# WdBlink/pyflyt-drone

Hardware: AMD Instinct MI355X
Metric: env-steps/sec at N parallel envs (FixedwingWaypoints) (higher is better)
Workload: dtype f64

## Files before the change

include/fwsim.h:

```cpp
#ifndef FWSIM_H
#define FWSIM_H

#include <stdint.h>

#ifdef __cplusplus
extern "C" {
#endif

#define FW_ABI_VERSION 7

#define FW_NUM_SURFACES 5
#define FW_NUM_ACTUATORS 6
#define FW_MAX_TARGETS 8
#define FW_MAX_COLLISION_PTS 8
#define FW_MAX_OBSTACLES 20
#define FW_VISION_FEATS 9
#define FW_VISION_HIST 3

enum {
  FW_OK = 0,
  FW_EINVAL = -1,
  FW_EHIP = -2,
  FW_ENOMEM = -3,
  FW_EVERSION = -4,
// ... 411 lines not shown
  void* act_env;
  float *rew_out, *start_out;
  void *obs, *reward;
  uint8_t *terminated, *truncated;
  void* terminal_obs;
  int32_t* info_i32;
  void* workspace; int64_t workspace_bytes;
  void* trace;
  double gamma;
  float clip_obs, eps_obs, clip_reward, eps_reward;
  int32_t update_obs, update_ret, norm_reward, deterministic;
} fw_collect_args;
int64_t fw_collect_step_workspace_bytes(fw_handle h);
int32_t fw_collect_workspace_init(fw_handle h, void* workspace, int64_t workspace_bytes, void* hip_stream);
int32_t fw_collect_step(fw_handle h, const fw_collect_args* a, void* hip_stream);
int32_t fw_collect_finish(fw_handle h, const fw_collect_args* a, void* hip_stream);
int32_t fw_collect_status(fw_handle h, const void* workspace, int64_t workspace_bytes, uint32_t* status_out, void* hip_stream);
typedef struct fw_collect_close_args {
  const float *rewards, *values, *episode_starts;
  float *adv, *ret;
  int32_t T;
  float gae_gamma, gae_lambda;
} fw_collect_close_args;
int32_t fw_collect_close(fw_handle h, const fw_collect_args* a, const fw_collect_close_args* c, void* hip_stream);

int32_t fw_num_envs(fw_handle h);
int32_t fw_lanes_per_env(fw_handle h);
int32_t fw_capture_wave(fw_handle h);
int32_t fw_axis_aligned(fw_handle h);
int32_t fw_aux_wave(fw_handle h);
int32_t fw_step_shape(fw_handle h);
enum {
  FW_PROBE_MATH1 = 0, FW_PROBE_MATH2 = 1, FW_PROBE_ROT = 2, FW_PROBE_EULER = 3, FW_PROBE_QUAT_STEP = 4, FW_PROBE_SURFACE = 5,
  FW_PROBE_GROUP = 6, FW_PROBE_RNG = 7, FW_PROBE_WIND = 8
};
enum { FW_PROBE_EULER_LANE = 0, FW_PROBE_EULER_LANES8 = 1, FW_PROBE_EULER_INVERSE = 2 };
enum { FW_PROBE_SURFACE_SCALAR = 0, FW_PROBE_SURFACE_REGS = 1, FW_PROBE_SURFACE_LDS = 2, FW_PROBE_SURFACE_AX = 3 };
enum { FW_PROBE_RNG_PHILOX = 0, FW_PROBE_RNG_UNIFORM = 1, FW_PROBE_RNG_NORMAL2 = 2 };
int32_t fw_probe(fw_handle h, int32_t op, int32_t variant, const double* in, int32_t in_cols, double* out, int32_t out_cols,
                 int32_t n, void* hip_stream);
typedef struct fw_sac_hyper {
  float lr, gamma, tau, beta1, beta2, eps, target_entropy, ent_coef;
  int32_t auto_ent, target_update_interval;
  uint64_t seed;
} fw_sac_hyper;
int32_t fw_sizeof_sac_hyper(void);
int32_t fw_sac_param_count(int32_t obs_dim, int32_t act_dim, int32_t hidden);
int64_t fw_sac_update_workspace_bytes(int32_t obs_dim, int32_t act_dim, int32_t hidden, int32_t batch);
int32_t fw_sac_act(const float* image, const void* obs, int32_t obs_is_f64, int32_t N, int32_t obs_dim, int32_t act_dim, int32_t hidden, int32_t mode,
                   uint64_t seed, int64_t env_offset, const int64_t* counters, float* act_f32, void* act_env, float* obs_stage, float* logp,
                   float* eps, void* hip_stream);
int32_t fw_replay_store(float* ring, int64_t capacity, int64_t* counters, const float* obs_stage, const float* act_f32, const void* reward,
                        const void* next_obs, const void* terminal_obs, const uint8_t* terminated, const uint8_t* truncated, int32_t env_is_f64,
                        int32_t N, int32_t obs_dim, int32_t act_dim, void* hip_stream);
int32_t fw_replay_sample(const float* ring, int64_t capacity, const int64_t* counters, uint64_t seed, int32_t row_floats, int32_t batch,
                         float* out, int32_t* idx_out, void* hip_stream);
int32_t fw_sac_noise(uint64_t seed, const int64_t* counters, int32_t batch, int32_t act_dim, float* out, void* hip_stream);
int32_t fw_sac_update(float* image, const float* batch_rows, int32_t obs_dim, int32_t act_dim, int32_t hidden, int32_t batch, const fw_sac_hyper* hyper,
                      int64_t* counters, float* out, void* workspace, int64_t workspace_bytes, void* hip_stream);
const char* fw_last_error(fw_handle h);
int32_t fw_destroy(fw_handle h);

#ifdef __cplusplus
}
#endif
#endif
```

pyflyt-drone_amd/csrc/fwsim.hip:

```cpp
#include <hip/hip_runtime.h>

#include <algorithm>
#include <cmath>
#include <cstdio>
#include <cstdlib>
#include <cstring>
#include <map>
#include <mutex>
#include <new>
#include <string>
#include <type_traits>
#include <vector>

#include "fwsim_device.hpp"
#include "fwsim_rollout.hpp"
#include "fwsim_ppo.hpp"
#include "fwsim_collect.hpp"
#include "fwsim_fused.hpp"
#include "fwsim_objlock.hpp"
#include "fwsim_render.hpp"

using namespace fwsim;


// ... 4 lines not shown
  for (int f = 0; f < RF_COUNT; ++f) D.r[tile_index(tile, RF_COUNT, f, env)] = (T)0;
  D.r[tile_index(tile, RF_COUNT, RF_QUAT + 3, env)] = (T)1;
  for (int f = 0; f < IF_COUNT; ++f) D.i[tile_index(tile, IF_COUNT, f, env)] = 0;
  D.i[tile_index(tile, IF_COUNT, IF_FLAGS, env)] = FL_TERM;
  D.i[tile_index(tile, IF_COUNT, IF_EPISODE, env)] = -1;
}

template <typename T>
__global__ void fw_warm_kernel(Params<T>* Pm) {
  if (threadIdx.x != 0 || blockIdx.x != 0) return;
  const Params<T>& P = *Pm;
  Rigid<T> S;
  for (int k = 0; k < 3; ++k) { S.p[k] = P.start_pos[k]; S.v[k] = P.start_vel[k]; S.w[k] = (T)0; }
  for (int k = 0; k < 4; ++k) S.q[k] = P.start_quat[k];
  for (int k = 0; k < FW_NUM_ACTUATORS; ++k) S.act[k] = (T)0;
  T cmd0[FW_NUM_ACTUATORS] = {(T)0, (T)0, (T)0, (T)0, (T)0, (T)0};
  T wind0[3] = {(T)0, (T)0, (T)0};
  int ticks = P.warmup_aviary_steps * P.ticks_per_aviary;
  TickC<T> C; SurfC<T> mine; T wmask;
  load_tick_constants<T, 1>(Pm, C, mine, wmask);
  T R[9];
  normalize_quat<T>(S.q);
  rot_from_unit_quat<T>(S.q, R);
  LaneAct<T> LA; LA.a = (T)0; LA.cmd = (T)0;
  for (int t = 0; t < ticks; ++t) (void)physics_tick<T, false, 1>(P, C, S, R, cmd0, (T)0, wind0, mine, wmask, LA);
  for (int k = 0; k < 3; ++k) { Pm->warm[k] = S.p[k]; Pm->warm[7 + k] = S.v[k]; Pm->warm[10 + k] = S.w[k]; }
  for (int k = 0; k < 4; ++k) Pm->warm[3 + k] = S.q[k];
  for (int k = 0; k < FW_NUM_ACTUATORS; ++k) Pm->warm[13 + k] = S.act[k];
  Pm->warm_ticks = ticks;
  const T a0[4] = {(T)0, (T)0, (T)0, (T)0};
  T Rw[9];
  (void)write_obs_attitude<T, false>(P, S, a0, Rw, [&](int k, T v) { Pm->warm_obs[k] = v; });
  for (int k = 0; k < 9; ++k) Pm->warm_R[k] = Rw[k];
}

__device__ __forceinline__ void pf_issue(double& dst, const double* p) { asm volatile("global_load_dwordx2 %0, %1, off" : "=v"(dst) : "v"(p) : "memory"); }
__device__ __forceinline__ void pf_issue(float& dst, const float* p) { asm volatile("global_load_dword %0, %1, off" : "=v"(dst) : "v"(p) : "memory"); }
template <typename T> __device__ __forceinline__ void pf_wait(T& a, T& b, T& c, T& d) { asm volatile("s_waitcnt vmcnt(0)" : "+v"(a), "+v"(b), "+v"(c), "+v"(d) :: "memory"); }
template <typename T> __device__ __forceinline__ void pf_tie(T& a, T& b, T& c, T& d) { asm volatile("" : "+v"(a), "+v"(b), "+v"(c), "+v"(d)); }
template <typename T> __device__ __forceinline__ T vload(const T* p) { return *p; }

template <typename T, bool COH = false>
__device__ __forceinline__ void load_action(const DevState<T>& D, const T* actions, int env, int src, T a[4]) {
  const T* ap = actions + (size_t)env * 4;
#pragma unroll
  for (int k = 0; k < 4; ++k) {
    T cur = COH ? ld_coherent(ap + k) : ap[k], old = D.r[(size_t)(RF_ACTION + k) * D.npad + env];
    a[k] = (src == 0) ? cur : (src == 1) ? old : (T)0;
  }
}

template <typename T> __device__ __forceinline__ DevState<T> shadow_view(const DevState<T>& D) {
  DevState<T> V = D; V.r = D.rs; V.i = nullptr; return V;
}
__device__ __forceinline__ unsigned long long pack_done(uint32_t ep, uint32_t epoch, int done) {
  return ((unsigned long long)ep << 32) | ((unsigned long long)(epoch & 0xFFFFFFu) << 8) | (unsigned long long)(done & 0xFF);
}

template <typename T, int G, int TKIND>
__device__ __forceinline__ void shadow_worker(const Params<T>* __restrict__ Pp, const ObjC<T>* __restrict__ OCp, DevState<T> D, int blk, int max_chunk = 0) {
  constexpr bool OBJ = TKIND == FW_TASK_OBJLOCK, COMB = TKIND == FW_TASK_WAYPOINT_OBJLOCK, HASOBJ = OBJ || COMB;
  constexpr int EPW = kWave / G;
  const Params<T>& P = *Pp;
  const ObjC<T>& OC = *OCp;
  const int lane = threadIdx.x & (kWave - 1), sub = (G == 1) ? 0 : (lane & (G - 1)), row = lane / G;
  const bool leader = sub == 0;
// ... 181 lines not shown

  T* aux_nz = AUX ? reinterpret_cast<T*>(smem_raw + Dg.mbox_off) : nullptr;
  if constexpr (AUX) {
    if (threadIdx.x >= kWave) {
      const int32_t a_tick = D.i[IF_TICK * n + envc], a_episode = D.i[IF_EPISODE * n + envc], a_flags = D.i[IF_FLAGS * n + envc];
      T a_z0 = (T)0, a_z1 = (T)0;
      if (FW_SH(has_noise) && FW_SH(step_ratio) <= G && !(a_flags & (FL_TERM | FL_TRUNC)))
        rng_normal2<T>(P, (uint32_t)(P.env_offset + envc), (uint32_t)a_episode, (uint32_t)(a_tick / FW_SH(ticks_per_aviary)) + (uint32_t)sub, a_z0, a_z1);
      aux_nz[2 * lane] = a_z0; aux_nz[2 * lane + 1] = a_z1;
      __syncthreads();
      return;
    }
  }

  int32_t step_count = D.i[IF_STEP * n + envc];
  int32_t tick = D.i[IF_TICK * n + envc];
  int32_t episode = D.i[IF_EPISODE * n + envc];
  int32_t flags = D.i[IF_FLAGS * n + envc];
  int32_t num_reached = D.i[IF_NUM_REACHED * n + envc];
  constexpr bool LANE_T = DEFER && G == 8;
  T tmine[3] = {(T)0, (T)0, (T)0};
  T a_keep = (T)0;
  if (LANE_T) {
    if (sub < FW_SH(num_targets)) {
#pragma unroll
      for (int k = 0; k < 3; ++k) tmine[k] = D.r[(size_t)(RF_TARGETS + 3 * sub + k) * n + envc];
    }
    if (!COLLECT) a_keep = actions[(size_t)envc * 4 + (sub & 3)];
  }
  Rigid<T> S;
  load_rigid<T>(D, envc, S);
  T new_dist = D.r[RF_NEW_DIST * n + envc];
  T ep_return = D.r[RF_EP_RETURN * n + envc];
  TickC<T> C; SurfC<T> mine_regs; T wmask;
  load_tick_constants<T, G, DEFER && G == 8 && WPE == 1>(Pp, C, mine_regs, wmask);
  if (AX && sub >= FW_NUM_SURFACES) mine_regs.hra = (T)0;
  SurfC<T>& mine = mine_regs;

  normalize_quat<T>(S.q);
  T R[9];
  rot_from_unit_quat<T>(S.q, R);
  ObjState<T> O;
  const ObjC<T>& OC = *OCp;
  if (HASOBJ) { obj_load<T, OBJ>(D, envc, O); obj_update_near_mask<T, G>(P, OC, D, envc, O, S); }
  int32_t out_strike = 0;
  unsigned long long sh_req = ~0ull, sh_done = 0ull;
  if ((GENERAL || DEFER) && D.shadow_on) { sh_req = D.sreq[envc]; sh_done = D.sdone[envc]; }
  T wb[3] = {(T)0, (T)0, (T)0}, wa[3] = {(T)0, (T)0, (T)0}, wphase = (T)0;
  if (GENERAL) {
#pragma unroll
    for (int k = 0; k < 3; ++k) { wb[k] = D.r[(RF_WIND + k) * n + envc]; wa[k] = D.r[(RF_WIND + 3 + k) * n + envc]; }
    wphase = D.r[(RF_WIND + 6) * n + envc];
  }
  T gust[2] = {(T)0, (T)1};
  if (GENERAL) gust_init<T>(P, wphase, tick, gust);
  T rew = (T)-0.1;
  T cmd[FW_NUM_ACTUATORS];
  double c_ret = 0.0;
  if (COLLECT) {
    if (active && leader) c_ret = ld_sc1(CAp->S.returns + env);
    collect_wait_actions(*CAp, Dg.epoch, env0, min(EPW, Dg.n - env0));
  }
  {
    const T* ap = actions + (size_t)envc * 4;
    T a4[4];
    if (COLLECT) collect_load_actions<T>(*CAp, ap, a4);
    else {
#pragma unroll
      for (int k = 0; k < 4; ++k) a4[k] = ap[k];
    }
    if (COLLECT && LANE_T) a_keep = (sub & 3) == 0 ? a4[0] : (sub & 3) == 1 ? a4[1] : (sub & 3) == 2 ? a4[2] : a4[3];
    const T sp[4] = { a4[0], a4[1], a4[2], a4[3] * (T)0.5 + (T)0.5 };
#pragma unroll
    for (int c = 0; c < FW_NUM_ACTUATORS; ++c)
      cmd[c] = P.mixer[c][0] * sp[0] + P.mixer[c][1] * sp[1] + P.mixer[c][2] * sp[2] + P.mixer[c][3] * sp[3];
  }
  LaneAct<T> LA; LA.a = (T)0; LA.cmd = (T)0;
  T cmd_mine = (T)0;
  if (G == 8) { lane_act_scatter<T>(S, LA); cmd_mine = lane_pick5<T>(cmd[0], cmd[1], cmd[2], cmd[3], cmd[4]); LA.cmd = cmd_mine; }

  T tcur[3] = {(T)0, (T)0, (T)0}, tnext[3] = {(T)0, (T)0, (T)0};
  const int gbase = lane & ~(G - 1);
  if (LANE_T) {
#pragma unroll
    for (int k = 0; k < 3; ++k) tcur[k] = __shfl(tmine[k], gbase | (num_reached & (G - 1)), kWave);
  } else if (!OBJ) {
    const int i0 = min(num_reached, FW_MAX_TARGETS - 1), i1 = min(num_reached + 1, FW_MAX_TARGETS - 1);
#pragma unroll
    for (int k = 0; k < 3; ++k) {
      tcur[k] = D.r[(size_t)(RF_TARGETS + 3 * i0 + k) * n + envc];
      tnext[k] = D.r[(size_t)(RF_TARGETS + 3 * i1 + k) * n + envc];
    }
  }

  const uint32_t genv = (uint32_t)(P.env_offset + envc);
  const bool done_at_entry = (flags & (FL_TERM | FL_TRUNC)) != 0;
  int tgt_obs = (flags >> FL_TGT_SHIFT) & 15;
  flags &= FL_MASK;
  int act_src = done_at_entry ? 1 : 0;

  const uint32_t astep0 = (uint32_t)(tick / FW_SH(ticks_per_aviary));
  const bool pre_noise = (G == 8) && FW_SH(has_noise) && (FW_SH(step_ratio) <= G);
  T nz0 = (T)0, nz1 = (T)0;
  if (!AUX && pre_noise && !done_at_entry) rng_normal2<T>(P, genv, (uint32_t)episode, astep0 + (uint32_t)sub, nz0, nz1);

  int phase = active ? PH_STEP : PH_DONE;
  constexpr bool STASH = (!DEFER && !HASOBJ) || COLLECT;
  double* latch = STASH ? reinterpret_cast<double*>(smem_raw + Dg.stash_off) : nullptr;
  int it = 0, warm_left = 0;
  const Mbox<T> MB = mbox_at<T>(HELP ? Dg.mbox_off : 0);
  uint32_t n_posted = 0, pend_seq = 0;
  int pend = 0;
// ... 1356 lines not shown
  O.near_ = (T)c.camera_near; O.far_ = (T)c.camera_far;
  O.inv_near = (T)(1.0 / c.camera_near); O.inv_far = (T)(1.0 / c.camera_far); O.db_c1 = (T)(c.camera_far / (c.camera_far - c.camera_near));
  O.zrow_stride = zrow_stride_of(res);
  O.duck_radius = (T)(c.duck_radius_per_scale * c.duck_global_scaling); O.half_dome = (T)(c.flight_dome_size / 2.0);
  O.obst_radius = (T)c.obstacle_radius; O.obst_hmin = (T)c.obstacle_height_range[0]; O.obst_hmax = (T)c.obstacle_height_range[1];
  O.safe_dist = (T)c.obstacle_safe_distance_m; O.avoid_scale = (T)c.obstacle_avoid_reward_scale; O.avoid_max = (T)c.obstacle_avoid_max_penalty;
  O.k_dist = (T)c.duck_distance_reward_scale; O.lock_radius = (T)c.duck_lock_center_radius; O.k_center = (T)c.duck_centering_reward_scale;
  O.k_visible = (T)c.duck_visible_step_reward; O.k_area = (T)c.duck_area_reward_scale; O.lost_penalty = (T)c.duck_lock_lost_penalty;
  O.approach_clip = (T)c.duck_approach_reward_clip_m; O.k_approach = (T)c.duck_approach_reward_scale;
  O.strike_dist = (T)c.duck_strike_distance_m; O.strike_reward = (T)c.duck_strike_reward; O.lock_step_reward = (T)c.duck_lock_step_reward;
  O.hold_steps = c.duck_lock_hold_steps; O.decay_steps = c.duck_lock_decay_steps; O.num_obstacles = c.num_obstacles;
  O.camera_ratio_ticks = (c.physics_hz / c.control_hz) * c.duck_camera_capture_interval_steps;
  O.switch_min_area = (T)c.duck_switch_min_area; O.switch_min_seen = c.duck_switch_min_consecutive_seen;
  {
    double rm = 0.0;
    for (int i = 0; i < c.n_collision_pts; ++i) { const double* q = c.collision_pts[i]; rm = std::max(rm, std::sqrt(q[0] * q[0] + q[1] * q[1] + q[2] * q[2])); }
    O.reach_margin = (T)(rm + 0.25);
  }
}

template <typename T>
int upload_params(fw_env* h) {
  Params<T> P;
  if (!build_params<T>(h->cfg, h->seed, h->env_offset, P, h->err)) return FW_EINVAL;
  if (!h->params_dev) HIP_TRY(h, hipMalloc(&h->params_dev, sizeof(Params<T>)));
  HIP_TRY(h, hipMemcpy(h->params_dev, &P, sizeof P, hipMemcpyHostToDevice));
  ObjC<T> OC;
  build_objc<T>(h->cfg, OC);
  if (!h->objc_dev) HIP_TRY(h, hipMalloc(&h->objc_dev, sizeof(ObjC<T>)));
  HIP_TRY(h, hipMemcpy(h->objc_dev, &OC, sizeof OC, hipMemcpyHostToDevice));
  if (P.warm_valid) {
    hipLaunchKernelGGL(fw_warm_kernel<T>, dim3(1), dim3(kWave), 0, 0, (Params<T>*)h->params_dev);
    HIP_TRY(h, hipGetLastError());
    HIP_TRY(h, hipDeviceSynchronize());
  }
  return FW_OK;
}

constexpr int kAny = -1;
struct KernelKey { int task, lanes, waves, windy, axis_aligned, capture_wave, aux_wave, step_shape; };
struct KernelRow { KernelKey key; EnvKernel step, reset, collect; };
template <typename... A> const void* kfn(void (*kernel)(A...)) { return (const void*)kernel; }
template <typename T> using StepFn = void (*)(const Params<T>*, const ObjC<T>*, DevState<T>, const T*, T*, T*, uint8_t*, uint8_t*, T*, int32_t*);
template <typename T> using CollectFn = void (*)(const Params<T>*, const ObjC<T>*, DevState<T>, const T*, T*, T*, uint8_t*, uint8_t*, T*, int32_t*, CollectArgs);
template <typename T> using ResetFn = void (*)(const Params<T>*, const ObjC<T>*, DevState<T>, const uint8_t*, T*, int, ScenOv);
template <typename T> using ResetLLFn = void (*)(const Params<T>*, DevState<T>, const uint8_t*, T*, int, ScenOv);
template <typename T> EnvKernel step_k(StepFn<T> f) { return {kfn(f)}; }
template <typename T> EnvKernel two_wave(StepFn<T> f) { return {kfn(f), 2 * kWave, false}; }
template <typename T> EnvKernel noise_wave(StepFn<T> f) { return {kfn(f), 2 * kWave, true}; }
template <typename T> EnvKernel collect_k(CollectFn<T> f) { return {kfn(f)}; }
template <typename T> EnvKernel reset_k(ResetFn<T> f) { return {kfn(f)}; }
template <typename T> EnvKernel no_objc(ResetLLFn<T> f) { return {kfn(f), kWave, true, false}; }
template <typename T> EnvKernel axis_aligned_step_kernel() {
  if constexpr (std::is_same<T, double>::value) return step_k<T>(fw_step_kernel_g8<T, false, true>); else return {};
}
template <typename T> EnvKernel aux_wave_step_kernel() {
  if constexpr (std::is_same<T, double>::value) return noise_wave<T>(fw_step_kernel_g8x<T>); else return {};
}
template <typename T> EnvKernel step_shape_step_kernel() {
  if constexpr (std::is_same<T, double>::value) return noise_wave<T>(fw_step_kernel_g8xs<T>); else return {};
}
template <typename T> const KernelRow* env_kernels_of(const KernelKey& q) {
  constexpr int LL = FW_TASK_LOWLEVEL, WD = FW_TASK_WAYPOINTS_DIRECT, OBJ = FW_TASK_OBJLOCK, COMB = FW_TASK_WAYPOINT_OBJLOCK, WP = FW_TASK_WAYPOINTS;
  static const KernelRow rows[] = {
    {{LL,   8, kAny, 1,    kAny, kAny, kAny, kAny}, step_k<T>(fw_step_kernel_ll<T, 8, true>),         no_objc<T>(fw_reset_kernel_ll<T, 8>),         {}},
    {{LL,   8, kAny, 0,    kAny, kAny, kAny, kAny}, step_k<T>(fw_step_kernel_ll<T, 8, false>),        no_objc<T>(fw_reset_kernel_ll<T, 8>),         {}},
    {{LL,   1, kAny, 1,    kAny, kAny, kAny, kAny}, step_k<T>(fw_step_kernel_ll<T, 1, true>),         no_objc<T>(fw_reset_kernel_ll<T, 1>),         {}},
    {{LL,   1, kAny, 0,    kAny, kAny, kAny, kAny}, step_k<T>(fw_step_kernel_ll<T, 1, false>),        no_objc<T>(fw_reset_kernel_ll<T, 1>),         {}},
// ... 1378 lines not shown
```

pyflyt-drone_amd/csrc/fwsim_device.hpp:

```cpp
#pragma once
#include <hip/hip_runtime.h>
#include <stdint.h>

#include "../../include/fwsim.h"

namespace fwsim {

constexpr int kWave = 64;
constexpr int kMaxObs = 64;

enum RF : int {
  RF_POS = 0, RF_QUAT = 3, RF_VEL = 7, RF_OMEGA = 10, RF_ACT = 13, RF_ACTION = 19,
  RF_NEW_DIST = 23, RF_WIND = 24, RF_EP_RETURN = 31, RF_TARGETS = 32,
  RF_TASK = 32 + 3 * FW_MAX_TARGETS,
  RF_COUNT = RF_TASK + (FW_STATE_DIM - FW_S_TASK)
};
enum IF : int { IF_STEP = 0, IF_TICK = 1, IF_EPISODE = 2, IF_FLAGS = 3, IF_NUM_REACHED = 4, IF_COUNT = 5 };

enum Flags : int { FL_TERM = 1, FL_TRUNC = 2, FL_COLLISION = 4, FL_OOB = 8, FL_COMPLETE = 16, FL_MASK = 0xFF, FL_TGT_SHIFT = 8 };

template <typename T>
struct SurfC {
  T dt_tau;
  T lift[3], fwd[3], pos[3], tq[3];
// ... 8 lines not shown
  T defl_scale;
  T k_exp;
};

template <typename T>
struct Params {
  SurfC<T> s[FW_NUM_SURFACES];
  T motor_dt_tau, noise_ratio;
  T m_force[3], m_torque[3], m_pos[3];
  T m_wrench_t[3];
  T mixer[FW_NUM_ACTUATORS][4];
  T inv_mass, gravity;
  T I[9], Iinv[9];
  T coll[FW_MAX_COLLISION_PTS][3];
  T dt, inv_physics_hz, physics_hz_T;
  T dome, reach, min_height, spawn_hi;
  T start_pos[3], start_quat[4], start_vel[3];
  T wind_base[3], wind_amp[3], wind_phase, gust_omega, wind_force_coef;
  T gust_sd, gust_cd;
  double wind_base_range[3][2], wind_amp_range[3][2];
  T warm[19];
  T warm_obs[24], warm_R[9];
  int32_t warm_valid, warm_ticks;
  int32_t n_coll, gyroscopic;
  int32_t task, angle_repr, att_dim, obs_dim, ctx;
  int32_t num_targets, sparse, auto_reset;
  int32_t max_steps, step_ratio, ticks_per_aviary, warmup_aviary_steps;
  int32_t wind_mode, wind_randomize, wind_randomize_phase, wind_coupling;
  int32_t has_noise;
  uint32_t seed_lo, seed_hi;
  int64_t env_offset;
  double ll_speed[2], ll_height[2];
  int32_t ll_max_steps;
};

struct ShapeOfParams {
  static constexpr bool kFixed = false;
  static constexpr int kTickUnroll = 1, kCtxUnroll = 1;
  static constexpr int step_ratio = -1, ticks_per_aviary = -1, ctx = -1, num_targets = -1, obs_dim = -1, att_dim = -1, sparse = -1,
                       angle_repr = -1, has_noise = -1, gyroscopic = -1, task = -1;
};
#ifndef FW_SHAPE_TICK_UNROLL
#define FW_SHAPE_TICK_UNROLL 2
#endif
#ifndef FW_SHAPE_CTX_UNROLL
#define FW_SHAPE_CTX_UNROLL 1
#endif
struct ShapeTrainWaypoints {
  static constexpr bool kFixed = true;
  static constexpr int kTickUnroll = FW_SHAPE_TICK_UNROLL, kCtxUnroll = FW_SHAPE_CTX_UNROLL;
  static constexpr int step_ratio = 4, ticks_per_aviary = 2, ctx = 2, num_targets = 8, obs_dim = 28, att_dim = 22, sparse = 1,
                       angle_repr = 0, has_noise = 1, gyroscopic = 1, task = FW_TASK_WAYPOINTS;
};
#define FW_SH(field) (SH::kFixed ? (int)SH::field : (int)P.field)
__device__ __forceinline__ double sum_squares_fma(double x, double y, double z) { return __builtin_fma(z, z, __builtin_fma(y, y, x * x)); }
__device__ __forceinline__ void mtv_fma(const double m[9], const double v[3], double o[3]) {
#pragma unroll
  for (int i = 0; i < 3; ++i) o[i] = __builtin_fma(m[i + 6], v[2], __builtin_fma(m[i + 3], v[1], m[i] * v[0]));
}

template <typename T>
struct DevState {
  T* r;
  int32_t* i;
  int32_t n, npad;
  T* rs;
// ... 400 lines not shown
  if (P.wind_mode == FW_WIND_CONSTANT) { w[0] = wb[0]; w[1] = wb[1]; w[2] = wb[2]; return; }
  T t = (T)tick * P.inv_physics_hz;
  T s = M<T>::sin_(P.gust_omega * t + phase);
  w[0] = wb[0] + wa[0] * s; w[1] = wb[1] + wa[1] * s; w[2] = wb[2] + wa[2] * s;
}

template <typename T>
__device__ __forceinline__ void gust_init(const Params<T>& P, T phase, int32_t tick, T g[2]) {
  g[0] = (T)0; g[1] = (T)1;
  if (P.wind_mode == FW_WIND_GUST_SINE) M<T>::sincos_(P.gust_omega * ((T)tick * P.inv_physics_hz) + phase, &g[0], &g[1]);
}
template <typename T>
__device__ __forceinline__ void gust_advance(const Params<T>& P, T g[2]) {
  const T s = g[0] * P.gust_cd + g[1] * P.gust_sd, c = g[1] * P.gust_cd - g[0] * P.gust_sd;
  g[0] = s; g[1] = c;
}
template <typename T>
__device__ __forceinline__ void wind_from_phase(const Params<T>& P, const T wb[3], const T wa[3], const T g[2], T w[3]) {
  if (P.wind_mode == FW_WIND_OFF) { w[0] = w[1] = w[2] = (T)0; return; }
  if (P.wind_mode == FW_WIND_CONSTANT) { w[0] = wb[0]; w[1] = wb[1]; w[2] = wb[2]; return; }
  w[0] = wb[0] + wa[0] * g[0]; w[1] = wb[1] + wa[1] * g[0]; w[2] = wb[2] + wa[2] * g[0];
}

template <typename T>
struct TickC {
  T dt_tau[FW_NUM_SURFACES];
  T motor_dt_tau, noise_ratio;
  T mF[3], mT[3];
  T inv_mass, gravity, dt, hdt;
  T I[9], Iinv[9];
  T wind_force_coef;
  T cpt[3];
  T cvalid;
};

__device__ __forceinline__ int opaque_zero() {
  int z;
  asm volatile("v_mov_b32 %0, 0" : "=v"(z));
  return z;
}

template <typename T, int G, bool RESIDENT = (G == 8)>
__device__ __forceinline__ void load_tick_constants(const Params<T>* Pp, TickC<T>& C, SurfC<T>& mine, T& wmask) {
  const int sub = (G == 1) ? 0 : (int)(threadIdx.x & (G - 1));
  const Params<T>* Q = (G == 1 || !RESIDENT) ? Pp : Pp + opaque_zero();
#pragma unroll
  for (int s = 0; s < FW_NUM_SURFACES; ++s) C.dt_tau[s] = Q->s[s].dt_tau;
  C.motor_dt_tau = Q->motor_dt_tau; C.noise_ratio = Q->noise_ratio;
#pragma unroll
  for (int k = 0; k < 3; ++k) { C.mF[k] = Q->m_force[k]; C.mT[k] = Q->m_wrench_t[k]; }
  C.inv_mass = Q->inv_mass; C.gravity = Q->gravity; C.dt = Q->dt; C.hdt = (T)0.5 * Q->dt;
#pragma unroll
  for (int k = 0; k < 9; ++k) { C.I[k] = Q->I[k]; C.Iinv[k] = Q->Iinv[k]; }
  C.wind_force_coef = Q->wind_force_coef;
  const int ci = (G == 1) ? 0 : sub;
#pragma unroll
  for (int k = 0; k < 3; ++k) C.cpt[k] = Q->coll[ci][k];
  C.cvalid = (ci < Q->n_coll) ? (T)1 : (T)0;
  mine = Q->s[(G == 1) ? 0 : min(sub, FW_NUM_SURFACES - 1)];
  wmask = (sub < FW_NUM_SURFACES) ? (T)1 : (T)0;
}

template <typename T>
__device__ __forceinline__ void rot_from_unit_quat(const T q[4], T m[9]) {
  T x = q[0], y = q[1], z = q[2], w = q[3];
  T xs = x + x, ys = y + y, zs = z + z;
  T wx = w * xs, wy = w * ys, wz = w * zs, xx = x * xs, xy = x * ys, xz = x * zs, yy = y * ys, yz = y * zs, zz = z * zs;
  m[0] = (T)1 - (yy + zz); m[1] = xy - wz;           m[2] = xz + wy;
  m[3] = xy + wz;           m[4] = (T)1 - (xx + zz); m[5] = yz - wx;
  m[6] = xz - wy;           m[7] = yz + wx;           m[8] = (T)1 - (xx + yy);
}
template <typename T>
__device__ __forceinline__ void rot_from_unit_quat_fma(const T q[4], T m[9]) {
  T x = q[0], y = q[1], z = q[2], w = q[3];
  T xs = x + x, ys = y + y, zs = z + z;
  T wx = w * xs, wy = w * ys, wz = w * zs, yy = y * ys, zz = z * zs;
  m[0] = (T)1 - __builtin_fma(y, ys, zz); m[1] = __builtin_fma(x, ys, -wz);       m[2] = __builtin_fma(x, zs, wy);
  m[3] = __builtin_fma(x, ys, wz);        m[4] = (T)1 - __builtin_fma(x, xs, zz); m[5] = __builtin_fma(y, zs, -wx);
  m[6] = __builtin_fma(x, zs, -wy);       m[7] = __builtin_fma(y, zs, wx);        m[8] = (T)1 - __builtin_fma(x, xs, yy);
}
template <typename T>
__device__ __forceinline__ void normalize_quat(T q[4]) {
  T d = q[0] * q[0] + q[1] * q[1] + q[2] * q[2] + q[3] * q[3];
  if (M<T>::fabs_(d - (T)1) > (T)1e-12) {
    T inv = M<T>::rcp_(M<T>::sqrt_(d));
    q[0] *= inv; q[1] *= inv; q[2] *= inv; q[3] *= inv;
  }
}

template <typename T> struct LaneAct { T a, cmd; };
template <typename T>
__device__ __forceinline__ T lane_pick5(T v0, T v1, T v2, T v3, T v4) {
  const int sub = threadIdx.x & 7;
  T a = v0;
  a = (sub == 1) ? v1 : a; a = (sub == 2) ? v2 : a; a = (sub == 3) ? v3 : a; a = (sub >= 4) ? v4 : a;
  return a;
}
template <typename T> __device__ __forceinline__ void lane_act_scatter(const Rigid<T>& S, LaneAct<T>& LA) {
  LA.a = lane_pick5<T>(S.act[0], S.act[1], S.act[2], S.act[3], S.act[4]);
}
template <typename T>
__device__ __forceinline__ void lane_act_gather(Rigid<T>& S, const LaneAct<T>& LA) {
  const int gbase = threadIdx.x & ~7;
#pragma unroll
  for (int k = 0; k < FW_NUM_SURFACES; ++k) S.act[k] = __shfl(LA.a, gbase | k, kWave);
}

template <typename T>
__device__ __forceinline__ void tick_actuators(const TickC<T>& C, Rigid<T>& S, const T cmd[FW_NUM_ACTUATORS], T noise_z) {
#pragma unroll
  for (int s = 0; s < FW_NUM_SURFACES; ++s) S.act[s] += C.dt_tau[s] * (cmd[s] - S.act[s]);
  T thr = S.act[FW_NUM_SURFACES];
  thr += C.motor_dt_tau * (cmd[FW_NUM_SURFACES] - thr);
  thr += noise_z * thr * C.noise_ratio;
  S.act[FW_NUM_SURFACES] = thr;
}

template <typename T>
__device__ __forceinline__ void quat_integrate(const TickC<T>& C, Rigid<T>& S) {
  const T dt = C.dt, hdt = C.hdt;
  T w2 = S.w[0] * S.w[0] + S.w[1] * S.w[1] + S.w[2] * S.w[2];
  T x = w2 * hdt * hdt;
  T x2 = x * x, x4 = x2 * x2;
  T s01 = (T)1 + x * (T)(-1.0 / 6.0), s23 = (T)(1.0 / 120.0) + x * (T)(-1.0 / 5040.0);
  T s45 = (T)(1.0 / 362880.0) + x * (T)(-1.0 / 39916800.0), s67 = (T)(1.0 / 6227020800.0) + x * (T)(-1.0 / 1307674368000.0);
  T sinc = (s01 + s23 * x2) + (s45 + s67 * x2) * x4;
  T c01 = (T)1 + x * (T)-0.5, c23 = (T)(1.0 / 24.0) + x * (T)(-1.0 / 720.0);
  T c45 = (T)(1.0 / 40320.0) + x * (T)(-1.0 / 3628800.0), c67 = (T)(1.0 / 479001600.0) + x * (T)(-1.0 / 87178291200.0);
  T ch = (c01 + c23 * x2) + (c45 + c67 * x2 + (T)(1.0 / 20922789888000.0) * x4) * x4;
  T k = sinc * hdt;
  const T lim = (T)(0.25 * kPi);
  if (w2 * dt * dt > lim * lim) {
    T ang = M<T>::div_(lim, dt);
    T sh;
    M<T>::sincos_((T)0.5 * ang * dt, &sh, &ch);
    k = M<T>::div_(sh, ang);
  }
  T ax = S.w[0] * k, ay = S.w[1] * k, az = S.w[2] * k;
  T qx = S.q[0], qy = S.q[1], qz = S.q[2], qw = S.q[3];
  T nx = ch * qx + ax * qw + ay * qz - az * qy;
  T ny = ch * qy + ay * qw + az * qx - ax * qz;
  T nz = ch * qz + az * qw + ax * qy - ay * qx;
  T nw = ch * qw - ax * qx - ay * qy - az * qz;
  T n2 = (nx * nx + ny * ny) + (nz * nz + nw * nw);
  T e = n2 - (T)1;
  T e2 = e * e;
  T inv = ((T)1 + e * (T)-0.5) + e2 * (((T)0.375 + e * (T)-0.3125) + e2 * (T)0.2734375);
  if (M<T>::fabs_(e) >= (T)1e-4) inv = M<T>::rcp_(M<T>::sqrt_(n2));
  S.q[0] = nx * inv; S.q[1] = ny * inv; S.q[2] = nz * inv; S.q[3] = nw * inv;
}

template <typename T, bool WIND, int G, bool AX = false, typename SH = ShapeOfParams, typename SC>
__device__ __forceinline__ bool physics_tick(const Params<T>& P, const TickC<T>& C, Rigid<T>& S, T R[9],
                                             const T cmd[FW_NUM_ACTUATORS], T noise_z, const T wind[3],
                                             SC& mine, T wmask, LaneAct<T>& LA) {
  if (G == 8) {
    LA.a += mine.dt_tau * (LA.cmd - LA.a);
    T thr = S.act[FW_NUM_SURFACES];
    thr += C.motor_dt_tau * (cmd[FW_NUM_SURFACES] - thr);
    thr += noise_z * thr * C.noise_ratio;
    S.act[FW_NUM_SURFACES] = thr;
  } else {
    tick_actuators<T>(C, S, cmd, noise_z);
  }
  T v_b[3], w_b[3], wind_b[3] = {(T)0, (T)0, (T)0};
  if constexpr (SH::kFixed) { mtv_fma(R, S.v, v_b); mtv_fma(R, S.w, w_b); }
  else { mtv(R, S.v, v_b); mtv(R, S.w, w_b); }
  if (WIND && P.wind_coupling == FW_WIND_COUPLE_AIRSPEED) mtv(R, wind, wind_b);
  T F[3] = {(T)0, (T)0, (T)0}, Tq[3] = {(T)0, (T)0, (T)0};
// ... 17 lines not shown
      surface_wrench<T, const SurfC<T>>(P.s[s], a_s, v_b, w_b, wind_b, f, tq);
#pragma unroll
      for (int k = 0; k < 3; ++k) { F[k] += f[k]; Tq[k] += tq[k]; }
    }
  }
  {
    T thr = S.act[FW_NUM_SURFACES];
    T t2 = thr * thr;
#pragma unroll
    for (int k = 0; k < 3; ++k) { F[k] += t2 * C.mF[k]; Tq[k] += t2 * C.mT[k]; }
  }
  const T dt = C.dt;
  T Fw[3];
  mv(R, F, Fw);
  if (WIND && P.wind_coupling == FW_WIND_COUPLE_FORCE) {
    Fw[0] += C.wind_force_coef * wind[0]; Fw[1] += C.wind_force_coef * wind[1]; Fw[2] += C.wind_force_coef * wind[2];
  }
  T acc[3] = { Fw[0] * C.inv_mass, Fw[1] * C.inv_mass, Fw[2] * C.inv_mass - C.gravity };
  T Iw[3], rhs[3] = { Tq[0], Tq[1], Tq[2] }, al_b[3], al_w[3];
  if (AX) { Iw[0] = C.I[0] * w_b[0]; Iw[1] = C.I[4] * w_b[1]; Iw[2] = C.I[8] * w_b[2]; }
  else mv(C.I, w_b, Iw);
  if (FW_SH(gyroscopic)) {
    T g[3];
    cross(w_b, Iw, g);
    rhs[0] -= g[0]; rhs[1] -= g[1]; rhs[2] -= g[2];
  }
  if (AX) { al_b[0] = C.Iinv[0] * rhs[0]; al_b[1] = C.Iinv[4] * rhs[1]; al_b[2] = C.Iinv[8] * rhs[2]; }
  else mv(C.Iinv, rhs, al_b);
  mv(R, al_b, al_w);
#pragma unroll
  for (int k = 0; k < 3; ++k) { S.v[k] += acc[k] * dt; S.w[k] += al_w[k] * dt; }
#pragma unroll
  for (int k = 0; k < 3; ++k) S.p[k] += S.v[k] * dt;
  quat_integrate<T>(C, S);
  if constexpr (SH::kFixed) rot_from_unit_quat_fma<T>(S.q, R); else rot_from_unit_quat<T>(S.q, R);
  bool contact = false;
  if (G == 8) {
    T zc = S.p[2] + R[6] * C.cpt[0] + R[7] * C.cpt[1] + R[8] * C.cpt[2];
    contact = group_any<8>(C.cvalid != (T)0 && zc <= (T)0);
  } else {
    for (int i = 0; i < P.n_coll; ++i) {
      T zc = S.p[2] + R[6] * P.coll[i][0] + R[7] * P.coll[i][1] + R[8] * P.coll[i][2];
      contact |= (zc <= (T)0);
    }
  }
  return contact;
}


template <typename T>
__device__ __forceinline__ bool euler_from_quat(const T q[4], T e[3]) {
  T x = q[0], y = q[1], z = q[2], w = q[3];
  T sarg = (T)-2 * (x * z - w * y);
  bool lock = (sarg <= (T)-0.99999) || (sarg >= (T)0.99999);
  if (lock) {
    bool neg = sarg <= (T)-0.99999;
    e[0] = (T)0;
    e[1] = neg ? (T)(-0.5 * kPi) : (T)(0.5 * kPi);
    e[2] = (T)2 * (neg ? M<T>::atan2_(x, -y) : M<T>::atan2_(-x, y));
  } else {
    T sqx = x * x, sqy = y * y, sqz = z * z, squ = w * w;
    e[0] = M<T>::atan2_((T)2 * (y * z + w * x), squ - sqx - sqy + sqz);
    e[1] = M<T>::asin_(sarg);
    e[2] = M<T>::atan2_((T)2 * (x * y + w * z), squ + sqx - sqy - sqz);
  }
  return lock;
}
// ... 239 lines not shown
```

pyflyt-drone_amd/csrc/fwsim_probe.hpp:

```cpp
#pragma once
#include <string>
#include <type_traits>

#include "fwsim_device.hpp"

namespace fwsim {
namespace probe {

struct Shape { int in_cols, out_cols, lanes_per_row; };
inline Shape shape_of(int op, int variant) {
  switch (op) {
    case FW_PROBE_MATH1: return variant == 0 ? Shape{1, 7, 1} : Shape{0, 0, 0};
    case FW_PROBE_MATH2: return variant == 0 ? Shape{2, 2, 1} : Shape{0, 0, 0};
    case FW_PROBE_ROT: return variant == 0 ? Shape{5, 23, 1} : Shape{0, 0, 0};
    case FW_PROBE_EULER:
      if (variant == FW_PROBE_EULER_LANE) return Shape{4, 4, 1};
      if (variant == FW_PROBE_EULER_LANES8) return Shape{4, 32, 8};
      if (variant == FW_PROBE_EULER_INVERSE) return Shape{3, 4, 1};
      return Shape{0, 0, 0};
    case FW_PROBE_QUAT_STEP: return variant == 0 ? Shape{7, 4, 1} : Shape{0, 0, 0};
    case FW_PROBE_SURFACE:
      if (variant == FW_PROBE_SURFACE_SCALAR) return Shape{11, 6, 1};
      if (variant == FW_PROBE_SURFACE_REGS || variant == FW_PROBE_SURFACE_LDS || variant == FW_PROBE_SURFACE_AX) return Shape{11, 6, 8};
      return Shape{0, 0, 0};
    case FW_PROBE_GROUP: return variant == 0 ? Shape{16, 80, 8} : Shape{0, 0, 0};
    case FW_PROBE_RNG:
      if (variant == FW_PROBE_RNG_PHILOX) return Shape{6, 4, 1};
      if (variant == FW_PROBE_RNG_UNIFORM) return Shape{5, 1, 1};
      if (variant == FW_PROBE_RNG_NORMAL2) return Shape{4, 2, 1};
      return Shape{0, 0, 0};
    case FW_PROBE_WIND: return variant == 0 ? Shape{9, 6, 1} : Shape{0, 0, 0};
    default: return Shape{0, 0, 0};
  }
}

template <typename T, int OP, int V>
__global__ __launch_bounds__(kWave) void fw_probe_kernel(const Params<T>* __restrict__ Pp, const double* __restrict__ in, double* __restrict__ out, int n) {
  constexpr int LPR = (OP == FW_PROBE_GROUP || (OP == FW_PROBE_EULER && V == FW_PROBE_EULER_LANES8) ||
                       (OP == FW_PROBE_SURFACE && V != FW_PROBE_SURFACE_SCALAR)) ? 8 : 1;
  const Params<T>& P = *Pp;
  const int gid = blockIdx.x * kWave + threadIdx.x;
  const int row = gid / LPR, sub = gid % LPR;
  const int rowc = row < n ? row : n - 1;
  const bool live = row < n;
  (void)sub; (void)P;

  if constexpr (OP == FW_PROBE_MATH1) {
    const double* x = in + (size_t)rowc;
    double* o = out + (size_t)rowc * 7;
    const T a = (T)x[0];
    T s, c;
    M<T>::sincos_(a, &s, &c);
    const T r0 = M<T>::rcp_(a), r1 = M<T>::sqrt_(a), r2 = M<T>::sin_(a), r5 = M<T>::asin_(a), r6 = M<T>::log_(a);
    if (live) { o[0] = (double)r0; o[1] = (double)r1; o[2] = (double)r2; o[3] = (double)s; o[4] = (double)c; o[5] = (double)r5; o[6] = (double)r6; }
  } else if constexpr (OP == FW_PROBE_MATH2) {
    const double* x = in + (size_t)rowc * 2;
    double* o = out + (size_t)rowc * 2;
    const T a = (T)x[0], b = (T)x[1];
    const T r0 = M<T>::div_(a, b), r1 = M<T>::atan2_(a, b);
    if (live) { o[0] = (double)r0; o[1] = (double)r1; }
  } else if constexpr (OP == FW_PROBE_ROT) {
    const double* x = in + (size_t)rowc * 5;
    double* o = out + (size_t)rowc * 23;
    T q[4] = { (T)x[0], (T)x[1], (T)x[2], (T)x[3] };
// ... 108 lines not shown
    philox4x32_10((uint32_t)x[0], (uint32_t)x[1], (uint32_t)x[2], (uint32_t)x[3], (uint32_t)x[4], (uint32_t)x[5], r);
    if (live) {
#pragma unroll
      for (int k = 0; k < 4; ++k) o[k] = (double)r[k];
    }
  } else if constexpr (OP == FW_PROBE_RNG && V == FW_PROBE_RNG_UNIFORM) {
    const double* x = in + (size_t)rowc * 5;
    const double u = rng_uniform<T>(P, (uint32_t)x[0], (uint32_t)x[1], (uint32_t)x[2], x[3], x[4]);
    if (live) out[rowc] = u;
  } else if constexpr (OP == FW_PROBE_RNG) {
    const double* x = in + (size_t)rowc * 4;
    double* o = out + (size_t)rowc * 2;
    const uint64_t a = ((uint64_t)(uint32_t)x[0] << 32) | (uint32_t)x[1], b = ((uint64_t)(uint32_t)x[2] << 32) | (uint32_t)x[3];
    T z0, z1;
    normal2_from_words<T>(a, b, z0, z1);
    if (live) { o[0] = (double)z0; o[1] = (double)z1; }
  } else if constexpr (OP == FW_PROBE_WIND) {
    const double* x = in + (size_t)rowc * 9;
    double* o = out + (size_t)rowc * 6;
    const T wb[3] = { (T)x[0], (T)x[1], (T)x[2] }, wa[3] = { (T)x[3], (T)x[4], (T)x[5] };
    const T phase = (T)x[6];
    const int32_t tick = (int32_t)x[7];
    int k = (int)x[8];
    k = k < 0 ? 0 : (k > 64 ? 64 : k);
    T g[2], w1[3], w2[3];
    gust_init<T>(P, phase, tick, g);
    for (int i = 0; i < k; ++i) gust_advance<T>(P, g);
    wind_from_phase<T>(P, wb, wa, g, w1);
    wind_at<T>(P, wb, wa, phase, tick + k, w2);
    if (live) {
#pragma unroll
      for (int i = 0; i < 3; ++i) { o[i] = (double)w1[i]; o[3 + i] = (double)w2[i]; }
    }
  }
}

template <typename T, int OP, int V>
inline hipError_t launch(const void* params_dev, const double* in, double* out, int n, hipStream_t stream) {
  const Shape sh = shape_of(OP, V);
  const long long threads = (long long)n * sh.lanes_per_row;
  const unsigned grid = (unsigned)((threads + kWave - 1) / kWave);
  hipLaunchKernelGGL((fw_probe_kernel<T, OP, V>), dim3(grid), dim3(kWave), 0, stream, (const Params<T>*)params_dev, in, out, n);
  return hipGetLastError();
}

template <typename T>
inline int dispatch(int op, int variant, bool axis_ok, const void* params_dev, const double* in, double* out, int n, hipStream_t stream,
                    hipError_t& herr, std::string& err) {
  herr = hipSuccess;
#define FW_PROBE_CASE(OP, V) if (op == (OP) && variant == (V)) { herr = launch<T, (OP), (V)>(params_dev, in, out, n, stream); return FW_OK; }
  FW_PROBE_CASE(FW_PROBE_MATH1, 0)
  FW_PROBE_CASE(FW_PROBE_MATH2, 0)
  FW_PROBE_CASE(FW_PROBE_ROT, 0)
  FW_PROBE_CASE(FW_PROBE_EULER, FW_PROBE_EULER_LANE)
  FW_PROBE_CASE(FW_PROBE_EULER, FW_PROBE_EULER_LANES8)
  FW_PROBE_CASE(FW_PROBE_EULER, FW_PROBE_EULER_INVERSE)
  FW_PROBE_CASE(FW_PROBE_QUAT_STEP, 0)
  FW_PROBE_CASE(FW_PROBE_SURFACE, FW_PROBE_SURFACE_SCALAR)
  FW_PROBE_CASE(FW_PROBE_SURFACE, FW_PROBE_SURFACE_REGS)
  FW_PROBE_CASE(FW_PROBE_SURFACE, FW_PROBE_SURFACE_LDS)
  if (op == FW_PROBE_SURFACE && variant == FW_PROBE_SURFACE_AX) {
    if constexpr (std::is_same<T, double>::value) {
      if (!axis_ok) { err = "fw_probe: the axis-aligned surface wrench needs a handle whose surfaces have forward = e_x, lift = e_y or e_z and a diagonal inertia"; return FW_EUNSUPPORTED; }
      herr = launch<T, FW_PROBE_SURFACE, FW_PROBE_SURFACE_AX>(params_dev, in, out, n, stream);
      return FW_OK;
    } else {
      err = "fw_probe: the axis-aligned surface wrench is built for float64 handles only";
      return FW_EUNSUPPORTED;
    }
  }
  FW_PROBE_CASE(FW_PROBE_GROUP, 0)
  FW_PROBE_CASE(FW_PROBE_RNG, FW_PROBE_RNG_PHILOX)
  FW_PROBE_CASE(FW_PROBE_RNG, FW_PROBE_RNG_UNIFORM)
  FW_PROBE_CASE(FW_PROBE_RNG, FW_PROBE_RNG_NORMAL2)
  FW_PROBE_CASE(FW_PROBE_WIND, 0)
#undef FW_PROBE_CASE
  err = "fw_probe: unknown (op, variant) = (" + std::to_string(op) + ", " + std::to_string(variant) + ")";
  return FW_EINVAL;
}

}
}
```

Measured before the change: 250.4 million.

## Precompute quaternion clamp constants and per-lane mixer row for fixed-shape step

Adds a one-time device kernel that computes the angular-rate clamp constants (cos/sinc terms) from dt and stores them in Params, so the fixed-shape quat integration reads them instead of calling sincos and divides each tick. In the fixed-shape path, each lane also loads its own mixer row and actions up front and computes only its surface command plus the motor command with FMAs, rather than all six rows followed by a lane pick. A probe op for checking the clamp constants is added. This trades a few extra registers and constant loads for less transcendental and mixer arithmetic per step.

```diff
diff --git a/include/fwsim.h b/include/fwsim.h
--- a/include/fwsim.h
+++ b/include/fwsim.h
@@ -467,11 +467,12 @@
 int32_t fw_step_shape(fw_handle h);
 enum {
   FW_PROBE_MATH1 = 0, FW_PROBE_MATH2 = 1, FW_PROBE_ROT = 2, FW_PROBE_EULER = 3, FW_PROBE_QUAT_STEP = 4, FW_PROBE_SURFACE = 5,
-  FW_PROBE_GROUP = 6, FW_PROBE_RNG = 7, FW_PROBE_WIND = 8
+  FW_PROBE_GROUP = 6, FW_PROBE_RNG = 7, FW_PROBE_WIND = 8, FW_PROBE_CLAMP = 9
 };
 enum { FW_PROBE_EULER_LANE = 0, FW_PROBE_EULER_LANES8 = 1, FW_PROBE_EULER_INVERSE = 2 };
 enum { FW_PROBE_SURFACE_SCALAR = 0, FW_PROBE_SURFACE_REGS = 1, FW_PROBE_SURFACE_LDS = 2, FW_PROBE_SURFACE_AX = 3 };
 enum { FW_PROBE_RNG_PHILOX = 0, FW_PROBE_RNG_UNIFORM = 1, FW_PROBE_RNG_NORMAL2 = 2 };
+enum { FW_PROBE_CLAMP_STORED = 0, FW_PROBE_CLAMP_FORMULA = 1 };
 int32_t fw_probe(fw_handle h, int32_t op, int32_t variant, const double* in, int32_t in_cols, double* out, int32_t out_cols,
                  int32_t n, void* hip_stream);
 typedef struct fw_sac_hyper {
diff --git a/pyflyt-drone_amd/csrc/fwsim.hip b/pyflyt-drone_amd/csrc/fwsim.hip
--- a/pyflyt-drone_amd/csrc/fwsim.hip
+++ b/pyflyt-drone_amd/csrc/fwsim.hip
@@ -60,6 +60,14 @@
   T Rw[9];
   (void)write_obs_attitude<T, false>(P, S, a0, Rw, [&](int k, T v) { Pm->warm_obs[k] = v; });
   for (int k = 0; k < 9; ++k) Pm->warm_R[k] = Rw[k];
+}
+
+template <typename T>
+__global__ void fw_clamp_kernel(Params<T>* Pm) {
+  if (threadIdx.x != 0 || blockIdx.x != 0) return;
+  T ch, k;
+  clamp_constants<T>(Pm->dt, ch, k);
+  Pm->clamp_ch = ch; Pm->clamp_k = k;
 }
 
 __device__ __forceinline__ void pf_issue(double& dst, const double* p) { asm volatile("global_load_dwordx2 %0, %1, off" : "=v"(dst) : "v"(p) : "memory"); }
@@ -307,6 +315,12 @@
   load_rigid<T>(D, envc, S);
   T new_dist = D.r[RF_NEW_DIST * n + envc];
   T ep_return = D.r[RF_EP_RETURN * n + envc];
+  T a4_first[4] = {(T)0, (T)0, (T)0, (T)0}, mix_mine[4] = {(T)0, (T)0, (T)0, (T)0};
+  if constexpr (SH::kFixed) {
+    const Params<T>* Qm = Pp + opaque_zero();
+#pragma unroll
+    for (int k = 0; k < 4; ++k) { a4_first[k] = actions[(size_t)envc * 4 + k]; mix_mine[k] = Qm->mixer[min(sub, FW_NUM_SURFACES - 1)][k]; }
+  }
   TickC<T> C; SurfC<T> mine_regs; T wmask;
   load_tick_constants<T, G, DEFER && G == 8 && WPE == 1>(Pp, C, mine_regs, wmask);
   if (AX && sub >= FW_NUM_SURFACES) mine_regs.hra = (T)0;
@@ -331,6 +345,7 @@
   if (GENERAL) gust_init<T>(P, wphase, tick, gust);
   T rew = (T)-0.1;
   T cmd[FW_NUM_ACTUATORS];
+  T cmd_mine = (T)0;
   double c_ret = 0.0;
   if (COLLECT) {
     if (active && leader) c_ret = ld_sc1(CAp->S.returns + env);
@@ -342,17 +357,24 @@
     if (COLLECT) collect_load_actions<T>(*CAp, ap, a4);
     else {
 #pragma unroll
-      for (int k = 0; k < 4; ++k) a4[k] = ap[k];
+      for (int k = 0; k < 4; ++k) a4[k] = SH::kFixed ? a4_first[k] : ap[k];
     }
     if (COLLECT && LANE_T) a_keep = (sub & 3) == 0 ? a4[0] : (sub & 3) == 1 ? a4[1] : (sub & 3) == 2 ? a4[2] : a4[3];
     const T sp[4] = { a4[0], a4[1], a4[2], a4[3] * (T)0.5 + (T)0.5 };
-#pragma unroll
-    for (int c = 0; c < FW_NUM_ACTUATORS; ++c)
-      cmd[c] = P.mixer[c][0] * sp[0] + P.mixer[c][1] * sp[1] + P.mixer[c][2] * sp[2] + P.mixer[c][3] * sp[3];
+    if constexpr (SH::kFixed) {
+      const auto mix_row = [&](T m0, T m1, T m2, T m3) { return __builtin_fma(m3, sp[3], __builtin_fma(m2, sp[2], __builtin_fma(m0, sp[0], m1 * sp[1]))); };
+#pragma unroll
+      for (int c = 0; c < FW_NUM_SURFACES; ++c) cmd[c] = (T)0;
+      cmd[FW_NUM_SURFACES] = mix_row(P.mixer[FW_NUM_SURFACES][0], P.mixer[FW_NUM_SURFACES][1], P.mixer[FW_NUM_SURFACES][2], P.mixer[FW_NUM_SURFACES][3]);
+      cmd_mine = mix_row(mix_mine[0], mix_mine[1], mix_mine[2], mix_mine[3]);
+    } else {
+#pragma unroll
+      for (int c = 0; c < FW_NUM_ACTUATORS; ++c)
+        cmd[c] = P.mixer[c][0] * sp[0] + P.mixer[c][1] * sp[1] + P.mixer[c][2] * sp[2] + P.mixer[c][3] * sp[3];
+    }
   }
   LaneAct<T> LA; LA.a = (T)0; LA.cmd = (T)0;
-  T cmd_mine = (T)0;
-  if (G == 8) { lane_act_scatter<T>(S, LA); cmd_mine = lane_pick5<T>(cmd[0], cmd[1], cmd[2], cmd[3], cmd[4]); LA.cmd = cmd_mine; }
+  if (G == 8) { lane_act_scatter<T>(S, LA); if (!SH::kFixed) cmd_mine = lane_pick5<T>(cmd[0], cmd[1], cmd[2], cmd[3], cmd[4]); LA.cmd = cmd_mine; }
 
   T tcur[3] = {(T)0, (T)0, (T)0}, tnext[3] = {(T)0, (T)0, (T)0};
   const int gbase = lane & ~(G - 1);
@@ -1775,8 +1797,10 @@
   if (P.warm_valid) {
     hipLaunchKernelGGL(fw_warm_kernel<T>, dim3(1), dim3(kWave), 0, 0, (Params<T>*)h->params_dev);
     HIP_TRY(h, hipGetLastError());
-    HIP_TRY(h, hipDeviceSynchronize());
-  }
+  }
+  hipLaunchKernelGGL(fw_clamp_kernel<T>, dim3(1), dim3(kWave), 0, 0, (Params<T>*)h->params_dev);
+  HIP_TRY(h, hipGetLastError());
+  HIP_TRY(h, hipDeviceSynchronize());
   return FW_OK;
 }
 
diff --git a/pyflyt-drone_amd/csrc/fwsim_device.hpp b/pyflyt-drone_amd/csrc/fwsim_device.hpp
--- a/pyflyt-drone_amd/csrc/fwsim_device.hpp
+++ b/pyflyt-drone_amd/csrc/fwsim_device.hpp
@@ -64,6 +64,7 @@
   int64_t env_offset;
   double ll_speed[2], ll_height[2];
   int32_t ll_max_steps;
+  T clamp_ch, clamp_k;
 };
 
 struct ShapeOfParams {
@@ -530,6 +531,7 @@
   T wind_force_coef;
   T cpt[3];
   T cvalid;
+  T clamp_ch, clamp_k;
 };
 
 __device__ __forceinline__ int opaque_zero() {
@@ -551,6 +553,7 @@
 #pragma unroll
   for (int k = 0; k < 9; ++k) { C.I[k] = Q->I[k]; C.Iinv[k] = Q->Iinv[k]; }
   C.wind_force_coef = Q->wind_force_coef;
+  C.clamp_ch = Q->clamp_ch; C.clamp_k = Q->clamp_k;
   const int ci = (G == 1) ? 0 : sub;
 #pragma unroll
   for (int k = 0; k < 3; ++k) C.cpt[k] = Q->coll[ci][k];
@@ -615,6 +618,15 @@
 }
 
 template <typename T>
+__device__ __forceinline__ void clamp_constants(T dt, T& ch, T& k) {
+  const T lim = (T)(0.25 * kPi);
+  T ang = M<T>::div_(lim, dt);
+  T sh;
+  M<T>::sincos_((T)0.5 * ang * dt, &sh, &ch);
+  k = M<T>::div_(sh, ang);
+}
+
+template <typename T, typename SH = ShapeOfParams>
 __device__ __forceinline__ void quat_integrate(const TickC<T>& C, Rigid<T>& S) {
   const T dt = C.dt, hdt = C.hdt;
   T w2 = S.w[0] * S.w[0] + S.w[1] * S.w[1] + S.w[2] * S.w[2];
@@ -629,10 +641,8 @@
   T k = sinc * hdt;
   const T lim = (T)(0.25 * kPi);
   if (w2 * dt * dt > lim * lim) {
-    T ang = M<T>::div_(lim, dt);
-    T sh;
-    M<T>::sincos_((T)0.5 * ang * dt, &sh, &ch);
-    k = M<T>::div_(sh, ang);
+    if constexpr (SH::kFixed) { ch = C.clamp_ch; k = C.clamp_k; }
+    else clamp_constants<T>(dt, ch, k);
   }
   T ax = S.w[0] * k, ay = S.w[1] * k, az = S.w[2] * k;
   T qx = S.q[0], qy = S.q[1], qz = S.q[2], qw = S.q[3];
@@ -716,7 +726,7 @@
   for (int k = 0; k < 3; ++k) { S.v[k] += acc[k] * dt; S.w[k] += al_w[k] * dt; }
 #pragma unroll
   for (int k = 0; k < 3; ++k) S.p[k] += S.v[k] * dt;
-  quat_integrate<T>(C, S);
+  quat_integrate<T, SH>(C, S);
   if constexpr (SH::kFixed) rot_from_unit_quat_fma<T>(S.q, R); else rot_from_unit_quat<T>(S.q, R);
   bool contact = false;
   if (G == 8) {
diff --git a/pyflyt-drone_amd/csrc/fwsim_probe.hpp b/pyflyt-drone_amd/csrc/fwsim_probe.hpp
--- a/pyflyt-drone_amd/csrc/fwsim_probe.hpp
+++ b/pyflyt-drone_amd/csrc/fwsim_probe.hpp
@@ -30,6 +30,7 @@
       if (variant == FW_PROBE_RNG_NORMAL2) return Shape{4, 2, 1};
       return Shape{0, 0, 0};
     case FW_PROBE_WIND: return variant == 0 ? Shape{9, 6, 1} : Shape{0, 0, 0};
+    case FW_PROBE_CLAMP: return (variant == FW_PROBE_CLAMP_STORED || variant == FW_PROBE_CLAMP_FORMULA) ? Shape{1, 2, 1} : Shape{0, 0, 0};
     default: return Shape{0, 0, 0};
   }
 }
@@ -204,6 +205,11 @@
 #pragma unroll
       for (int i = 0; i < 3; ++i) { o[i] = (double)w1[i]; o[3 + i] = (double)w2[i]; }
     }
+  } else if constexpr (OP == FW_PROBE_CLAMP) {
+    double* o = out + (size_t)rowc * 2;
+    T ch = P.clamp_ch, k = P.clamp_k;
+    if constexpr (V == FW_PROBE_CLAMP_FORMULA) clamp_constants<T>(P.dt, ch, k);
+    if (live) { o[0] = (double)ch; o[1] = (double)k; }
   }
 }
 
@@ -246,6 +252,8 @@
   FW_PROBE_CASE(FW_PROBE_RNG, FW_PROBE_RNG_UNIFORM)
   FW_PROBE_CASE(FW_PROBE_RNG, FW_PROBE_RNG_NORMAL2)
   FW_PROBE_CASE(FW_PROBE_WIND, 0)
+  FW_PROBE_CASE(FW_PROBE_CLAMP, FW_PROBE_CLAMP_STORED)
+  FW_PROBE_CASE(FW_PROBE_CLAMP, FW_PROBE_CLAMP_FORMULA)
 #undef FW_PROBE_CASE
   err = "fw_probe: unknown (op, variant) = (" + std::to_string(op) + ", " + std::to_string(variant) + ")";
   return FW_EINVAL;
```

New measurement: 252.7 million, median of 5. No clear change (+0.9%).
